# DhayaaAnbajagane/Baryonification

Hardware: AMD Instinct MI355X
Metric: halos/sec for BaryonifyShell NSIDE=1024 (1000000-halo synthetic catalog) (higher is better)
Workload: dtype f64 throughout in the parity-grade mode: f64 ring-row geometry, f64 pair math with 1e-11 elementary functions (fp32 seeds + one Newton step), f64 LDS accumulation, pix_offsets stored as two f32 arrays (hi + lo), f64 regrid geometry, f64 map

## Files before the change

### baryonification_amd/csrc/bfgx_kernels.hpp

```cpp
#pragma once
#include <hip/hip_runtime.h>
#include <stdint.h>
#include "bfgx_cosmo.hpp"
#include "bfgx_math.hpp"

namespace bfgx {

constexpr double kTwoPi    = 6.283185307179586476925286766559005768394;
constexpr double kHalfPi   = 1.570796326794896619231321691639751442099;
constexpr double kInvTwoPi = 1.0 / kTwoPi;
constexpr double kTwoThird = 2.0 / 3.0;
constexpr double kDeg2Rad  = kPi / 180.0;
constexpr double kRad2Deg  = 180.0 / kPi;

constexpr int kWave = 64;
constexpr int kWavesPerBlock = 4;
constexpr int kNC = 4;

enum { MODE_OFFSETS = 0, MODE_PAINT = 1, MODE_COUNT = 2 };

struct Hpx {
    int64_t nside, npix, ncap;
    double fact1, fact2;
};
// ... 3 lines not shown
    Hpx h;
    h.nside = nside;
    h.npix = 12 * nside * nside;
    h.ncap = 2 * nside * (nside - 1);
    h.fact2 = 4.0 / (double)h.npix;
    h.fact1 = (double)(nside << 1) * h.fact2;
    return h;
}

__device__ inline int64_t ring_above(const Hpx &h, double z)
{
    const double az = fabs(z);
    if (az <= kTwoThird) return (int64_t)((double)h.nside * (2.0 - 1.5 * z));
    const int64_t iring = (int64_t)((double)h.nside * sqrt(3.0 * (1.0 - az)));
    return (z > 0) ? iring : 4 * h.nside - iring - 1;
}

__device__ inline void ring_info_small(const Hpx &h, int64_t ring, int64_t &start, int64_t &nr, bool &shifted)
{
    if (ring < h.nside) {
        shifted = true; nr = 4 * ring; start = 2 * ring * (ring - 1);
    } else if (ring < 3 * h.nside) {
        shifted = ((ring - h.nside) & 1) == 0; nr = 4 * h.nside; start = h.ncap + (ring - h.nside) * nr;
    } else {
        const int64_t q = 4 * h.nside - ring;
        shifted = true; nr = 4 * q; start = h.npix - 2 * q * (q + 1);
    }
}

__device__ inline void ring_info2(const Hpx &h, int64_t ring, int64_t &start, int64_t &nr, double &theta, bool &shifted)
// ... 13 lines not shown

__device__ inline void ring_z_sth(const Hpx &h, int64_t ring, double &z, double &sth)
{
    if (ring < h.nside) {
        const double tmp = (double)(ring * ring) * h.fact2;
        z = 1.0 - tmp;
        sth = (z > 0.99) ? sqrt(tmp * (2.0 - tmp)) : sqrt((1.0 - z) * (1.0 + z));
    } else if (ring <= 3 * h.nside) {
        z = (double)(2 * h.nside - ring) * h.fact1;
        sth = sqrt((1.0 - z) * (1.0 + z));
    } else {
        const int64_t q = 4 * h.nside - ring;
        const double tmp = (double)(q * q) * h.fact2;
        z = tmp - 1.0;
        sth = (z < -0.99) ? sqrt(tmp * (2.0 - tmp)) : sqrt((1.0 - z) * (1.0 + z));
    }
}

__device__ inline int64_t isqrt64(int64_t v) { return (int64_t)sqrt((double)v + 0.5); }

__device__ inline void pix2loc(const Hpx &h, int64_t pix, double &z, double &sth, double &phi)
{
    if (pix < h.ncap) {
        const int64_t iring = (1 + isqrt64(1 + 2 * pix)) >> 1;
        const int64_t iphi = (pix + 1) - 2 * iring * (iring - 1);
        const double tmp = (double)(iring * iring) * h.fact2;
        z = 1.0 - tmp;
        sth = (z > 0.99) ? sqrt(tmp * (2.0 - tmp)) : sqrt((1.0 - z) * (1.0 + z));
        phi = ((double)iphi - 0.5) * kHalfPi / (double)iring;
    } else if (pix < h.npix - h.ncap) {
// ... 115 lines not shown
    if (!(dphi > 0.0)) return;
    const double sh = s.shifted ? 0.5 : 0.0;
    const double fnr = (double)s.nr * kInvTwoPi;
    const int64_t ip_lo = (int64_t)floor(fnr * (phi0 - dphi) - sh) + 1;
    const int64_t ip_hi = (int64_t)floor(fnr * (phi0 + dphi) - sh);
    int64_t c = ip_hi - ip_lo + 1;
    c = c < 0 ? 0 : (c > s.nr ? s.nr : c);
    s.cnt = (int)c;
    int64_t l = ip_lo;
    if (l < 0) l += s.nr;
    if (l >= s.nr) l -= s.nr;
    if (l < 0) l += s.nr;
    s.lo = (int)l;
}

__device__ inline void interp_neighbours(const Hpx &h, double theta, double phi, int32_t ring[4], int32_t k[4])
{
    int64_t pix[4]; double w[4];
    get_interpol<false>(h, theta, phi, pix, w);
    const double z = cos(theta);
    const int64_t ir1 = ring_above(h, z), ir2 = ir1 + 1;
    for (int q = 0; q < 4; ++q) {
        int64_t rg = (q < 2) ? ir1 : ir2;
        if (rg < 1) rg = 1;
        if (rg > 4 * h.nside - 1) rg = 4 * h.nside - 1;
        int64_t st, nr; bool sh;
        ring_info_small(h, rg, st, nr, sh);
        ring[q] = (int32_t)rg;
        k[q] = (int32_t)(pix[q] - st);
    }
}

struct DevTable {
    int32_t ndim;
    int32_t n[BFGX_MAX_DIM];
    const double *axis[BFGX_MAX_DIM];
// ... 69 lines not shown
    if (md.rho_type == 1) rho = b.rho_crit0 * b.Omega_m / (a * a * a);
    return cbrt(M / (4.18879020479 * md.Delta * rho));
}

__device__ inline int axis_find(const double *g, int n, double x)
{
    if (!(x >= g[0]) || !(x <= g[n - 1])) return -1;
    int lo = 0, hi = n - 1;
    while (hi - lo > 1) {
        const int mid = (lo + hi) >> 1;
        if (x >= g[mid]) lo = mid; else hi = mid;
    }
    return lo;
}

template <int NC>
__device__ inline bool table_corners(const DevTable &tab, const double *gz, const double *gm, double x0, double x1, const double *xe,
                                     double *wv, int32_t *ro)
{
    const int iz = axis_find(gz, tab.n[0], x0);
    const int im = axis_find(gm, tab.n[1], x1);
    constexpr int K = (NC == 4) ? 0 : (NC == 8 ? 1 : (NC == 16 ? 2 : (NC == 32 ? 3 : 4)));
    static_assert(NC == (4 << K), "NC = 4 * 2^K");
    int ip[K > 0 ? K : 1];
    double tp[K > 0 ? K : 1];
    bool oob = (iz < 0 || im < 0);
#pragma unroll
    for (int k = 0; k < K; ++k) {
        const double *g = tab.axis[3 + k];
        ip[k] = axis_find(g, tab.n[3 + k], xe[k]);
        tp[k] = 0.0;
        oob = oob || ip[k] < 0;
        if (ip[k] >= 0) tp[k] = (xe[k] - g[ip[k]]) / (g[ip[k] + 1] - g[ip[k]]);
    }
    if (!oob) {
        const double tz = (x0 - gz[iz]) / (gz[iz + 1] - gz[iz]);
        const double tm = (x1 - gm[im]) / (gm[im + 1] - gm[im]);
        const int nr = tab.n[2];
        for (int c = 0; c < NC; ++c) {
            const int bz = (c >> (K + 1)) & 1, bm = (c >> K) & 1;
            double w = (1.0 * (bz ? tz : 1.0 - tz)) * (bm ? tm : 1.0 - tm);
            int idx = (iz + bz) * tab.n[1] + im + bm;
#pragma unroll
            for (int k = 0; k < K; ++k) {
                const int b = (c >> (K - 1 - k)) & 1;
                w *= (b ? tp[k] : 1.0 - tp[k]);
                idx = idx * tab.n[3 + k] + ip[k] + b;
            }
            wv[c] = w;
            ro[c] = idx * nr;
        }
    } else {
        for (int c = 0; c < NC; ++c) { wv[c] = 0.0; ro[c] = 0; }
    }
    return oob;
}

struct Tiling {
    int32_t BR, W, nbands, ntiles;
    const int32_t *band_tile0;
    const int32_t *band_nphi;
    const int32_t *band_nrmin;
    const int32_t *tile_band;
    const int32_t *tile_order;
};

__device__ inline int tile_ks(int j, int nr, int nphi) { return (int)(((unsigned)j * (unsigned)nr + (unsigned)nphi - 1u) / (unsigned)nphi); }

__device__ inline int ring_len(const Hpx &h, int ring)
{
// ... 12 lines not shown
    int32_t _pad[2];
};

enum { kClsNone = 0, kClsNarrow = 1, kClsWide = 2 };

struct DiscSpan {
    int32_t fb, rfirst, rlast, allphi;
    int32_t fb_ring[4], fb_k[4];
    double flo, fhi;
};

template <typename F>
__device__ inline void for_each_tile(const Hpx &h, const Tiling &T, const DiscSpan &r, F &&f)
{
    if (r.fb) {
        int seen[4], ns = 0;
        for (int q = 0; q < 4; ++q) {
            const int b = (r.fb_ring[q] - 1) / T.BR;
            const int nphi = T.band_nphi[b];
            const int t = T.band_tile0[b] + (int)(((int64_t)r.fb_k[q] * nphi) / ring_len(h, r.fb_ring[q]));
            bool dup = false;
            for (int i = 0; i < ns; ++i) dup |= (seen[i] == t);
            if (!dup) { seen[ns++] = t; f(t); }
        }
        return;
    }
    if (r.rlast < r.rfirst) return;
    const int b0 = (r.rfirst - 1) / T.BR, b1 = (r.rlast - 1) / T.BR;
    for (int b = b0; b <= b1; ++b) {
        const int nphi = T.band_nphi[b], t0 = T.band_tile0[b];
        bool all = r.allphi || nphi == 1;
        int jlo = 0, jhi = nphi - 1;
        if (!all) {
            const double margin = 2.0 * (double)nphi / (double)T.band_nrmin[b] + 1e-6;
            jlo = (int)floor((double)nphi * r.flo - margin);
            jhi = (int)floor((double)nphi * r.fhi + margin);
            if (jhi - jlo + 1 >= nphi) { all = true; jlo = 0; jhi = nphi - 1; }
        }
        for (int jj = jlo; jj <= jhi; ++jj) {
            int j = jj % nphi;
            if (j < 0) j += nphi;
            f(t0 + j);
        }
    }
}

struct alignas(16) RowRec {
    double z0, s0, xa, cosr, phi0;
    int32_t rfirst, rlast;
    int32_t fb;
    int32_t _pad;
    double cut2;
};
struct FbRec { int32_t ring[4], k[4]; };

template <typename real>
struct alignas(16) PairRecT {
// ... 45 lines not shown
    RowRec *rowrec;
    void *pairrec;
    FbRec *fbrec;
    TileRef *tref;
    int32_t *cnt_a, *cnt_b, *cnt_w;
    int32_t *entries_a, *slow_list, *slow_cnt;
    float *work_est;
    int32_t cap_a;
    int32_t cnt_pad;
    int32_t fast;
    int32_t rec_all;
    int32_t ncell_m, nrm1;
    int64_t blk_rows, blk_stride;
};

template <int NC, typename real>
__device__ __forceinline__ void halo_prep_one(const DevModel &m, const Hpx &h, int64_t j, bool live, const double *gz, const double *gm,
                                              const double *__restrict__ M, const double *__restrict__ z,
                                              const double *__restrict__ ra, const double *__restrict__ dec,
                                              ExtraCols ex,
                                              const double *__restrict__ lnz1, const double *__restrict__ lnM,
                                              int fallback4, const Tiling &T, const PrepOut &o, int *s_nslow, float *s_work);

constexpr int kK0Occ = 4;
template <int NC, typename real>
__global__ void __launch_bounds__(256, kK0Occ)
halo_prep_kernel(DevModel m, Hpx h, int64_t nhalo,
                 const double *__restrict__ M, const double *__restrict__ z,
                 const double *__restrict__ ra, const double *__restrict__ dec,
                 ExtraCols ex,
                 const double *__restrict__ lnz1, const double *__restrict__ lnM,
                 int fallback4, Tiling T, PrepOut o)
{
    __shared__ int s_nslow;
    __shared__ float s_work;
    if (threadIdx.x == 0) { s_nslow = 0; s_work = 0.0f; }
    constexpr int kAxisLds = 128;
    __shared__ double ax_lds[2 * kAxisLds];
    const bool ax_in_lds = m.tab.n[0] <= kAxisLds && m.tab.n[1] <= kAxisLds;
    if (ax_in_lds) {
        for (int i = threadIdx.x; i < m.tab.n[0]; i += blockDim.x) ax_lds[i] = m.tab.axis[0][i];
        for (int i = threadIdx.x; i < m.tab.n[1]; i += blockDim.x) ax_lds[kAxisLds + i] = m.tab.axis[1][i];
        __syncthreads();
    }
    const double *gz = ax_in_lds ? ax_lds : m.tab.axis[0], *gm = ax_in_lds ? ax_lds + kAxisLds : m.tab.axis[1];
    constexpr int kBandLds = 1024;
    __shared__ int32_t band_lds[3 * kBandLds + 1];
    if (o.tref && T.nbands <= kBandLds) {
        for (int i = threadIdx.x; i <= T.nbands; i += blockDim.x) band_lds[i] = T.band_tile0[i];
        for (int i = threadIdx.x; i < T.nbands; i += blockDim.x) { band_lds[kBandLds + 1 + i] = T.band_nphi[i]; band_lds[2 * kBandLds + 1 + i] = T.band_nrmin[i]; }
        __syncthreads();
        T.band_tile0 = band_lds; T.band_nphi = band_lds + kBandLds + 1; T.band_nrmin = band_lds + 2 * kBandLds + 1;
    }
    __syncthreads();
    const int64_t j = (int64_t)blockIdx.x * blockDim.x + threadIdx.x;
    halo_prep_one<NC, real>(m, h, j < nhalo ? j : nhalo - 1, j < nhalo, gz, gm, M, z, ra, dec, ex, lnz1, lnM, fallback4, T, o, &s_nslow, &s_work);
    if (o.slow_cnt) {
        __syncthreads();
        if (threadIdx.x == 0) o.slow_cnt[blockIdx.x] = s_nslow;
        if (threadIdx.x == 0 && o.work_est) o.work_est[blockIdx.x] = s_work;
    }
}

template <int NC, typename real>
__device__ __forceinline__ void halo_prep_one(const DevModel &m, const Hpx &h, int64_t j, bool live, const double *gz, const double *gm,
                                              const double *__restrict__ M, const double *__restrict__ z,
                                              const double *__restrict__ ra, const double *__restrict__ dec,
                                              ExtraCols ex,
                                              const double *__restrict__ lnz1, const double *__restrict__ lnM,
                                              int fallback4, const Tiling &T, const PrepOut &o, int *s_nslow, float *s_work)
{
    HaloRec r;
    const int64_t jin = o.blk_rows > 0 ? (j / o.blk_rows) * o.blk_stride + (j % o.blk_rows) : j;
    const double M_j = M[jin], z_j = z[jin];
    const double a = 1.0 / (1.0 + z_j);
    const double R = dev_radius(m.bg_runner, m.md_runner, M_j, a);
    double D;
    {
        int i = (int)floor(z_j / m.da_step);
        i = max(0, min(i, kDaKnots - 2));
        const double t = z_j - (double)i * m.da_step;
        const double *c = m.da_coef + 4 * i;
        D = ((c[0] * t + c[1]) * t + c[2]) * t + c[3];
    }
    const double radius = R * m.eps_runner / D;

    const double theta = kHalfPi - dec[jin] * kDeg2Rad;
    const double phi = ra[jin] * kDeg2Rad;
    double st, ct, sp, cp;
    sincos_bounded(theta, st, ct);
    sincos_bounded(phi, sp, cp);
    const double thq = theta;
    double phq = phi - kTwoPi * floor(phi * kInvTwoPi);
    if (phq >= kTwoPi) phq -= kTwoPi;
    if (st == 0.0) phq = 0.0;
    r.z0 = ct;
    r.s0 = st;
    r.xa = 1.0 / sqrt((1.0 - r.z0) * (1.0 + r.z0));
    r.phi0 = phq;
    r.cph0 = cp; r.sph0 = sp;
    r.theta = theta; r.phi = phi;
    r.D = D; r.a = a;

    const int64_t nl4 = 4 * h.nside;
    bool pole = false;
    double sr_ = 0.0;
    const bool bad = !live || !(radius > 0.0) || !isfinite(radius) || !(theta >= 0.0) || !(theta <= kPi) || !isfinite(phi);
    if (bad) {
        r.cosr = 1.0; r.irmin = 1; r.irmax = 0; r.rfirst = 1; r.rlast = 0;
        r.z0 = 1.0; r.s0 = 0.0; r.xa = 1.0; r.phi0 = 0.0; r.cph0 = 1.0; r.sph0 = 0.0;
    } else if (radius >= kPi) {
        r.cosr = -1.0; r.irmin = (int32_t)nl4; r.irmax = 0; r.rfirst = 1; r.rlast = (int32_t)(nl4 - 1);
        pole = true;
    } else {
        double cr_;
        sincos_bounded(radius, sr_, cr_);
        r.cosr = cr_;
        const double rlat1 = thq - radius;
        const double rlat2 = thq + radius;
        int64_t irmin = ring_above(h, ct * cr_ + st * sr_) + 1;
        int64_t irmax = ring_above(h, ct * cr_ - st * sr_);
        if (irmax > nl4 - 1) irmax = nl4 - 1;
        r.irmin = (int32_t)irmin; r.irmax = (int32_t)irmax;
        r.rfirst = (int32_t)(((rlat1 <= 0) && (irmin > 1)) ? 1 : irmin);
        r.rlast = (int32_t)(((rlat2 >= kPi) && (irmax + 1 < nl4)) ? nl4 - 1 : irmax);
        pole = (rlat1 <= 0) || (rlat2 >= kPi);
    }
    double dmax;
    {
        const double sr = (radius >= kHalfPi) ? 1.0 : sr_;
        r.allphi = (pole || radius >= kHalfPi || !(sr < 0.999 * r.s0)) ? 1 : 0;
        const double xs = sr / r.s0, xs2 = xs * xs;
        const double as_small = xs * (1.0 + xs2 * (1.0 / 6.0 + xs2 * (3.0 / 40.0 + xs2 * (15.0 / 336.0 + xs2 * (105.0 / 3456.0)))));
        dmax = r.allphi ? kPi : (xs < 0.35 ? as_small * (1.0 + 2e-6) : asin(xs));
        r.flo = (phq - dmax) * kInvTwoPi;
        r.fhi = (phq + dmax) * kInvTwoPi;
    }

    r.fb = 0; r._pad = 0;
    for (int q = 0; q < 4; ++q) { r.fb_ring[q] = 0; r.fb_k[q] = 0; }
    if (fallback4 && !bad && (r.rlast - r.rfirst) < 8) {
        int total = 0;
        const int span = r.rlast - r.rfirst, mid = (r.rfirst + r.rlast) >> 1;
        for (int t = 0; t <= span && total < 4; ++t) {
            const int ring = mid + ((t & 1) ? ((t + 1) >> 1) : -(t >> 1));
            RowSpan s;
            disc_row(h, ring, r.z0, r.xa, r.cosr, r.phi0, r.irmin, r.irmax, s);
            total += s.cnt;
        }
        if (total < 4) {
            r.fb = 1;
            interp_neighbours(h, theta, phi, r.fb_ring, r.fb_k);
        }
    }

    int cls = kClsWide;
    bool geo_wide = false;
    if (bad) cls = kClsNone;
    else if (o.fast && NC == 4 && !r.allphi && dmax <= 0.40) {
        cls = kClsNarrow;
        if (r.fb) for (int q = 0; q < 4; ++q) if (r.fb_ring[q] < 16 || r.fb_ring[q] > (int)nl4 - 16) cls = kClsWide;
    }
    if (o.fast == 2 && NC == 4 && cls == kClsWide) { cls = kClsNarrow; geo_wide = true; }
    if (o.work_est) {
        float w = (cls == kClsNarrow) ? (r.fb ? 4.0f : (float)(radius * radius) * 0.25f * (float)h.npix) : 0.0f;
#pragma unroll
        for (int sft = kWave >> 1; sft > 0; sft >>= 1) w += __shfl_xor(w, sft, kWave);
        if ((threadIdx.x & (kWave - 1)) == 0) atomicAdd(s_work, w);
    }
    TileRef ref;
    RunSlot run[kRefMax];
    for (int i = 0; i < kRefMax; ++i) { run[i].base = 0; run[i].hr = 0; }
    ref.n = 0; ref.cls = cls; ref._pad[0] = ref._pad[1] = 0;
    for (int i = 0; i < kRefMax; ++i) { ref.few.tile[i] = 0; ref.few.slot[i] = 0; }
    if (o.tref) {
        DiscSpan ds;
        ds.fb = r.fb; ds.rfirst = r.rfirst; ds.rlast = r.rlast; ds.allphi = r.allphi; ds.flo = r.flo; ds.fhi = r.fhi;
        for (int q = 0; q < 4; ++q) { ds.fb_ring[q] = r.fb_ring[q]; ds.fb_k[q] = r.fb_k[q]; }
        int tl[kRefMax] = {0, 0, 0, 0};
        int nt = 0;
        if (cls != kClsNone) for_each_tile(h, T, ds, [&](int t) { if (nt < kRefMax) tl[nt] = t; ++nt; });
        ref.n = nt; ref.cls = cls; ref._pad[0] = ref._pad[1] = 0;
#pragma unroll
        for (int i = 0; i < kRefMax; ++i) {
            run[i] = wave_run_issue(o.cnt_a, o.entries_a ? tl[i] * o.cnt_pad : tl[i], nt <= kRefMax && i < nt && cls == kClsNarrow);
            if (nt <= kRefMax) { ref.few.tile[i] = (i < nt) ? tl[i] : 0; ref.few.slot[i] = 0; }
        }
        if (nt <= kRefMax) {
            for (int i = 0; i < kRefMax; ++i)
                if (i < nt && cls != kClsNarrow) atomicAdd(o.cnt_w + tl[i], 1);
        } else {
            ref.many.rfirst = r.rfirst; ref.many.rlast = r.rlast; ref.many.allphi = r.allphi; ref.many._p = 0;
            ref.many.flo = r.flo; ref.many.fhi = r.fhi;
            int32_t *cnt = (cls == kClsNarrow) ? o.cnt_b : o.cnt_w;
            for_each_tile(h, T, ds, [&](int t) { atomicAdd(cnt + t, 1); });
        }
    }
    const double Rmod = (m.same_model ? R : dev_radius(m.bg_model, m.md_model, M_j, a)) / a;
    r.rcut = m.tab.eps_model * Rmod;
    r.inv_a = 1.0 / a;
    const double x0 = lnz1 ? lnz1[jin] : fast_log(1.0 / a), x1 = lnM ? lnM[jin] : fast_log(M_j);
    r.lnoff = m.tab.rdelta ? (x0 - fast_log(Rmod)) : x0;
    double wv[NC];
    int32_t ro[NC];
    double xe[BFGX_MAX_EXTRA];
#pragma unroll
    for (int k = 0; k < BFGX_MAX_EXTRA; ++k) xe[k] = ((4 << k) < NC) ? ex.p[k][jin] : 0.0;
    const bool oob = table_corners<NC>(m.tab, gz, gm, x0, x1, xe, wv, ro);
    r.oob = oob ? 1 : 0;
    if (NC == 4) {
        for (int c = 0; c < 4; ++c) { r.w[c] = wv[c]; r.rowoff[c] = ro[c]; }
    } else {
        for (int c = 0; c < 4; ++c) { r.w[c] = 0.0; r.rowoff[c] = 0; }
        RowSetX rx;
        for (int c = 0; c < kNCmaxShell; ++c) { rx.w[c] = c < NC ? wv[c] : 0.0; rx.rowoff[c] = c < NC ? ro[c] : 0; }
        if (live) o.rowsx[j] = rx;
    }

    if (live && o.rec && (o.rec_all || cls == kClsWide)) o.rec[j] = r;
    if (cls == kClsNarrow) {
        RowRec rr;
        rr.z0 = r.z0; rr.s0 = r.s0; rr.xa = r.xa; rr.cosr = r.cosr; rr.phi0 = r.phi0;
        rr.rfirst = r.rfirst; rr.rlast = r.rlast; rr.fb = (r.fb ? 1 : 0) | (geo_wide ? 2 : 0); rr._pad = 0;
        const double cut = r.rcut * a / D;
        rr.cut2 = cut * cut;
        double sh, chh;
        sincos_bounded(0.5 * fmin(radius, kPi), sh, chh);
        const bool implied = (m.tab.logv != 0) || (!r.fb && cut >= 2.0 * sh * (1.0 + 1e-9));
        o.rowrec[j] = rr;
        PairRecT<real> pr;
        double scl = D * r.inv_a;
        if (m.tab.rdelta) scl /= Rmod;
        pr.scale2 = oob ? (real)1.0e30 : (real)(scl * scl);
        pr.cut2 = implied ? (real)0 : (real)(1.0 / rr.cut2);
        pr.aD = (real)(a / D);
        pr.cph0 = (real)r.cph0; pr.sph0 = (real)r.sph0;
        for (int c = 0; c < 4; ++c) pr.w[c] = (real)wv[c < NC ? c : 0];
        const int nr = o.nrm1 + 1, nm = o.ncell_m + 1;
        const int row0 = oob ? 0 : ro[0] / nr;
        const int iz = row0 / nm, im = row0 - iz * nm;
        pr.cell = (iz * o.ncell_m + im) * o.nrm1 * 8;
        pr.oob = oob ? 1 : 0;
        pr.hidx = (int32_t)j; pr._pad = 0;
        reinterpret_cast<PairRecT<real> *>(o.pairrec)[j] = pr;
        if (r.fb || geo_wide) {
            FbRec f;
            for (int q = 0; q < 4; ++q) { f.ring[q] = r.fb_ring[q]; f.k[q] = r.fb_k[q]; }
            if (!r.fb) { f.ring[0] = r.irmin; f.ring[1] = r.irmax; }
            o.fbrec[j] = f;
        }
    }
    if (o.tref) {
#pragma unroll
        for (int i = 0; i < kRefMax; ++i) {
            const int sl = wave_run_resolve(run[i]);
            if (ref.n <= kRefMax && ref.cls == kClsNarrow && i < ref.n) ref.few.slot[i] = sl;
        }
        bool slow = (ref.cls != kClsNone) && (ref.n > kRefMax || ref.cls != kClsNarrow);
        if (ref.cls == kClsNarrow && ref.n <= kRefMax) {
            for (int i = 0; i < kRefMax; ++i) if (i < ref.n) {
                const int sl = ref.few.slot[i];
                if (o.entries_a && sl < o.cap_a) o.entries_a[(int64_t)ref.few.tile[i] * o.cap_a + sl] = (int32_t)j;
                else if (o.entries_a) { ref.few.slot[i] = -1; atomicAdd(o.cnt_b + ref.few.tile[i], 1); slow = true; }
                else slow = true;
            }
        }
        if (live && (slow || !o.slow_list)) o.tref[j] = ref;
        if (slow && o.slow_list) o.slow_list[(int64_t)blockIdx.x * 256 + atomicAdd(s_nslow, 1)] = (int32_t)j;
    }
}

__global__ void __launch_bounds__(256)
disc_rings_kernel(DevModel m, Hpx h, int64_t nhalo, const double *__restrict__ M, const double *__restrict__ z,
                  const double *__restrict__ dec, int32_t *__restrict__ rings, int margin)
{
    const int64_t j = (int64_t)blockIdx.x * blockDim.x + threadIdx.x;
    if (j >= nhalo) return;
    const double M_j = M[j], z_j = z[j];
    const double a = 1.0 / (1.0 + z_j);
    const double R = dev_radius(m.bg_runner, m.md_runner, M_j, a);
    double D;
    {
        int i = (int)floor(z_j / m.da_step);
        i = max(0, min(i, kDaKnots - 2));
        const double t = z_j - (double)i * m.da_step;
        const double *c = m.da_coef + 4 * i;
        D = ((c[0] * t + c[1]) * t + c[2]) * t + c[3];
    }
    const double radius = R * m.eps_runner / D;
    const double theta = kHalfPi - dec[j] * kDeg2Rad;
    const int nl4 = (int)(4 * h.nside);
    int first = 1, last = 0;
    const bool bad = !(radius > 0.0) || !isfinite(radius) || !(theta >= 0.0) || !(theta <= kPi) || !(M_j > 0.0) || !isfinite(M_j) || !(z_j > -1.0);
    if (!bad) {
        if (radius >= kPi) { first = 1; last = nl4 - 1; }
        else {
            const double lo = fmax(theta - radius, 0.0), hi = fmin(theta + radius, kPi);
            first = (int)ring_above(h, cos(lo)) - 1;
            last = (int)ring_above(h, cos(hi)) + 2;
            first = max(1, first - 1); last = min(nl4 - 1, last + 1);
        }
        first = max(1, first - margin); last = min(nl4 - 1, last + margin);
    }
    rings[2 * j] = first; rings[2 * j + 1] = last;
// ... 85 lines not shown
    }
}
__global__ void __launch_bounds__(256)
route_step_kernel(RouteStepArgs s, DevModel m, Hpx h, int64_t n, int32_t *__restrict__ cursor)
{
    const RouteArgs &a = s.r;
    __shared__ int hist[kRouteMaxRanks], base[kRouteMaxRanks], taken[kRouteMaxRanks];
    const int tid = threadIdx.x;
    if (tid < kRouteMaxRanks) { hist[tid] = 0; taken[tid] = 0; }
    __syncthreads();
    const int64_t per = (n + gridDim.x - 1) / gridDim.x;
    const int64_t j0 = (int64_t)blockIdx.x * per, j1 = min(n, j0 + per);
    const int nl4 = (int)(4 * h.nside);
    auto ring_range = [&](int64_t j, int &first, int &last) {
        const double M_j = s.M[j], z_j = s.z[j];
        const double aa = 1.0 / (1.0 + z_j);
        const double R = dev_radius(m.bg_runner, m.md_runner, M_j, aa);
        double D;
        {
            int i = (int)floor(z_j / m.da_step);
            i = max(0, min(i, kDaKnots - 2));
            const double t = z_j - (double)i * m.da_step;
            const double *c = m.da_coef + 4 * i;
            D = ((c[0] * t + c[1]) * t + c[2]) * t + c[3];
        }
        const double radius = R * m.eps_runner / D;
        const double theta = kHalfPi - s.dec[j] * kDeg2Rad;
        first = 1; last = 0;
        const bool bad = !(radius > 0.0) || !isfinite(radius) || !(theta >= 0.0) || !(theta <= kPi) || !(M_j > 0.0) || !isfinite(M_j) || !(z_j > -1.0);
        if (bad) return;
        if (radius >= kPi) { first = 1; last = nl4 - 1; }
        else {
            const double lo = fmax(theta - radius, 0.0), hi = fmin(theta + radius, kPi);
            first = (int)ring_above(h, cos(lo)) - 1;
            last = (int)ring_above(h, cos(hi)) + 2;
            first = max(1, first - 1); last = min(nl4 - 1, last + 1);
        }
        first = max(1, first - s.margin); last = min(nl4 - 1, last + s.margin);
    };
    constexpr int kStash = 4096;
    __shared__ int2 stash[kStash];
// ... 899 lines not shown
```

### baryonification_amd/csrc/bfgx_scatter2.hpp

```cpp
#pragma once
#include "bfgx_kernels.hpp"
#include <type_traits>

namespace bfgx {

constexpr int kW2 = 8;
constexpr int kChunk2 = 16;
constexpr int kPlanePad = 11;

template <typename real> struct PMath;
__device__ inline float fma_(float a, float b, float c) { return __builtin_fmaf(a, b, c); }
__device__ inline double fma_(double a, double b, double c) { return __builtin_fma(a, b, c); }

template <> struct PMath<float> {
    static constexpr float kHuge = 1.0e37f;
    static __device__ inline float rsq(float x) { return __builtin_amdgcn_rsqf(x); }
    static __device__ inline float half_ln(float x) { return 0.34657359027997264f * __builtin_amdgcn_logf(x); }
    static __device__ inline float expv(float d) { return __builtin_amdgcn_exp2f(d * 1.4426950408889634f); }
    static __device__ inline void sin_omc(float x, float &sn, float &omc)
    {
        const float u = x * x;
        float ps = -1.0f / 5040.0f;
        ps = __builtin_fmaf(ps, u, 1.0f / 120.0f);
        ps = __builtin_fmaf(ps, u, -1.0f / 6.0f);
// ... 110 lines not shown
    PairRecT<real> pair[K1Cfg<real>::chunk];
    RowC2<real> rows[K1Cfg<real>::rowl];
    unsigned long long mask[K1Cfg<real>::rowl + 4];
    EntC2 ent[K1Cfg<real>::chunk];
    unsigned long long emask[K1Cfg<real>::chunk];
};

template <typename real>
__host__ __device__ inline size_t tile2_lds_bytes(int BR, int W, int ncomp)
{
    size_t a = (size_t)ncomp * ((size_t)BR * W + kPlanePad) * sizeof(double);
    a = (a + 15) & ~(size_t)15;
    return a + sizeof(Wave2Lds<real>) * kW2 + 16 + (sizeof(TileRow) + sizeof(RingC2<real>)) * (size_t)BR;
}

__constant__ double kAtanS1[6] = {1.62858201153657823623e-02, 4.97687799461593236017e-02, 6.66107313738753120669e-02,
                                  9.09088713343650656196e-02, 1.42857142725034663711e-01, 3.33333333333329318027e-01};
__constant__ double kAtanS2[5] = {-3.65315727442169155270e-02, -5.83357013379057348645e-02, -7.69187620504482999495e-02,
                                  -1.11111104054623557880e-01, -1.99999999998764832476e-01};
template <bool CMEM = false>
__device__ inline double atan_lt_7_16(double t)
{
    const double z = t * t, w = z * z;
    if (CMEM) {
        double s1 = kAtanS1[0], s2 = kAtanS2[0];
#pragma unroll
        for (int k = 1; k < 6; ++k) s1 = __builtin_fma(s1, w, kAtanS1[k]);
#pragma unroll
        for (int k = 1; k < 5; ++k) s2 = __builtin_fma(s2, w, kAtanS2[k]);
        return __builtin_fma(-t, __builtin_fma(z, s1, w * s2), t);
    }
    double s1 = 1.62858201153657823623e-02;
    s1 = __builtin_fma(s1, w, 4.97687799461593236017e-02);
    s1 = __builtin_fma(s1, w, 6.66107313738753120669e-02);
    s1 = __builtin_fma(s1, w, 9.09088713343650656196e-02);
    s1 = __builtin_fma(s1, w, 1.42857142725034663711e-01);
    s1 = __builtin_fma(s1, w, 3.33333333333329318027e-01);
    double s2 = -3.65315727442169155270e-02;
    s2 = __builtin_fma(s2, w, -5.83357013379057348645e-02);
    s2 = __builtin_fma(s2, w, -7.69187620504482999495e-02);
    s2 = __builtin_fma(s2, w, -1.11111104054623557880e-01);
    s2 = __builtin_fma(s2, w, -1.99999999998764832476e-01);
    return __builtin_fma(-t, __builtin_fma(z, s1, w * s2), t);
}

template <bool CMEM = false>
__device__ inline void disc_row_span_narrow(int nr, bool shifted, double z, double fnr, double z0, double xa, double cosr,
                                            double phi0, int &lo, int &cnt)
{
    lo = 0; cnt = 0;
    const double x = (cosr - z * z0) * xa;
    const double ysq = 1.0 - z * z - x * x;
    if (!(ysq > 0.0) || !(x > 0.0)) return;
    const double t = ysq * fast_rsq(ysq) * fast_rcp(x);
    const double dphi = atan_lt_7_16<CMEM>(t);
    if (!(dphi > 0.0)) return;
    const double sh = shifted ? 0.5 : 0.0;
    const int ip_lo = (int)floor(fnr * (phi0 - dphi) - sh) + 1;
    const int ip_hi = (int)floor(fnr * (phi0 + dphi) - sh);
    cnt = max(0, min(ip_hi - ip_lo + 1, nr));
    int l = ip_lo;
    if (l < 0) l += nr;
    if (l >= nr) l -= nr;
    if (l < 0) l += nr;
    lo = l;
}

__device__ __noinline__ bool exact_cut_test(const TileRow &tr, const RowRec &rr, int kloc)
{
    const int kk = tr.ks + kloc;
    const double xx = fold_dphi(__builtin_fma((double)kk + (tr.shifted ? 0.5 : 0.0), tr.dphi, -rr.phi0));
    double sh, ch;
    if (fabs(xx) <= 1.0) sincos_small(0.5 * xx, sh, ch);
    else sincos_bounded(0.5 * xx, sh, ch);
    const double s2 = 2.0 * sh * ch, o2 = 2.0 * sh * sh;
    const double wx = (tr.sth - rr.s0) - tr.sth * o2, wy = tr.sth * s2, wz = tr.z - rr.z0;
    return (wx * wx + wy * wy + wz * wz) < rr.cut2;
}

__device__ __noinline__ int2 disc_row_span_wide(const TileRow &tr, int ring, const RowRec &rr, const FbRec &fr)
{
// ... 846 lines not shown
```

Baseline: 911.7 million.

## Compact fallback-candidate halos into LDS work lists in the halo prep kernel

Restructures the halo prep kernel so the few-pixel fallback census and interp_neighbours run only on halos compacted into block-level LDS lists via wave ballots. The per-thread divergent fallback path becomes dense lane work. Several smaller edits come with it: 32-bit ring math, deferring the phi sincos, writing NC>4 table corners straight to global memory, cheaper tile dedup and wrap in for_each_tile, and a small-angle sincos. The cost is a large LDS struct and three extra block barriers per prep block.

```diff
diff --git a/baryonification_amd/csrc/bfgx_kernels.hpp b/baryonification_amd/csrc/bfgx_kernels.hpp
--- a/baryonification_amd/csrc/bfgx_kernels.hpp
+++ b/baryonification_amd/csrc/bfgx_kernels.hpp
@@ -41,6 +41,14 @@
     if (az <= kTwoThird) return (int64_t)((double)h.nside * (2.0 - 1.5 * z));
     const int64_t iring = (int64_t)((double)h.nside * sqrt(3.0 * (1.0 - az)));
     return (z > 0) ? iring : 4 * h.nside - iring - 1;
+}
+
+__device__ inline int ring_above32(const Hpx &h, double z)
+{
+    const double az = fabs(z);
+    if (az <= kTwoThird) return (int)((double)h.nside * (2.0 - 1.5 * z));
+    const int iring = (int)((double)h.nside * sqrt(3.0 * (1.0 - az)));
+    return (z > 0) ? iring : 4 * (int)h.nside - iring - 1;
 }
 
 __device__ inline void ring_info_small(const Hpx &h, int64_t ring, int64_t &start, int64_t &nr, bool &shifted)
@@ -84,6 +92,21 @@
         const double tmp = (double)(q * q) * h.fact2;
         z = tmp - 1.0;
         sth = (z < -0.99) ? sqrt(tmp * (2.0 - tmp)) : sqrt((1.0 - z) * (1.0 + z));
+    }
+}
+
+__device__ inline void ring_len_z(const Hpx &h, int ring, int &nr, bool &shifted, double &z)
+{
+    const int ns = (int)h.nside;
+    if (ring < ns) {
+        const double tmp = ((double)ring * (double)ring) * h.fact2;
+        z = 1.0 - tmp; nr = 4 * ring; shifted = true;
+    } else if (ring <= 3 * ns) {
+        z = (double)(2 * ns - ring) * h.fact1; nr = 4 * ns; shifted = ((ring - ns) & 1) == 0;
+    } else {
+        const int q = 4 * ns - ring;
+        const double tmp = ((double)q * (double)q) * h.fact2;
+        z = tmp - 1.0; nr = 4 * q; shifted = true;
     }
 }
 
@@ -229,12 +252,64 @@
     s.lo = (int)l;
 }
 
-__device__ inline void interp_neighbours(const Hpx &h, double theta, double phi, int32_t ring[4], int32_t k[4])
+__constant__ double kAtanS1[6] = {1.62858201153657823623e-02, 4.97687799461593236017e-02, 6.66107313738753120669e-02,
+                                  9.09088713343650656196e-02, 1.42857142725034663711e-01, 3.33333333333329318027e-01};
+__constant__ double kAtanS2[5] = {-3.65315727442169155270e-02, -5.83357013379057348645e-02, -7.69187620504482999495e-02,
+                                  -1.11111104054623557880e-01, -1.99999999998764832476e-01};
+template <bool CMEM = false>
+__device__ inline double atan_lt_7_16(double t)
+{
+    const double z = t * t, w = z * z;
+    if (CMEM) {
+        double s1 = kAtanS1[0], s2 = kAtanS2[0];
+#pragma unroll
+        for (int k = 1; k < 6; ++k) s1 = __builtin_fma(s1, w, kAtanS1[k]);
+#pragma unroll
+        for (int k = 1; k < 5; ++k) s2 = __builtin_fma(s2, w, kAtanS2[k]);
+        return __builtin_fma(-t, __builtin_fma(z, s1, w * s2), t);
+    }
+    double s1 = 1.62858201153657823623e-02;
+    s1 = __builtin_fma(s1, w, 4.97687799461593236017e-02);
+    s1 = __builtin_fma(s1, w, 6.66107313738753120669e-02);
+    s1 = __builtin_fma(s1, w, 9.09088713343650656196e-02);
+    s1 = __builtin_fma(s1, w, 1.42857142725034663711e-01);
+    s1 = __builtin_fma(s1, w, 3.33333333333329318027e-01);
+    double s2 = -3.65315727442169155270e-02;
+    s2 = __builtin_fma(s2, w, -5.83357013379057348645e-02);
+    s2 = __builtin_fma(s2, w, -7.69187620504482999495e-02);
+    s2 = __builtin_fma(s2, w, -1.11111104054623557880e-01);
+    s2 = __builtin_fma(s2, w, -1.99999999998764832476e-01);
+    return __builtin_fma(-t, __builtin_fma(z, s1, w * s2), t);
+}
+
+template <bool CMEM = false>
+__device__ inline void disc_row_span_narrow(int nr, bool shifted, double z, double fnr, double z0, double xa, double cosr,
+                                            double phi0, int &lo, int &cnt)
+{
+    lo = 0; cnt = 0;
+    const double x = (cosr - z * z0) * xa;
+    const double ysq = 1.0 - z * z - x * x;
+    if (!(ysq > 0.0) || !(x > 0.0)) return;
+    const double t = ysq * fast_rsq(ysq) * fast_rcp(x);
+    const double dphi = atan_lt_7_16<CMEM>(t);
+    if (!(dphi > 0.0)) return;
+    const double sh = shifted ? 0.5 : 0.0;
+    const int ip_lo = (int)floor(fnr * (phi0 - dphi) - sh) + 1;
+    const int ip_hi = (int)floor(fnr * (phi0 + dphi) - sh);
+    cnt = max(0, min(ip_hi - ip_lo + 1, nr));
+    int l = ip_lo;
+    if (l < 0) l += nr;
+    if (l >= nr) l -= nr;
+    if (l < 0) l += nr;
+    lo = l;
+}
+
+__device__ inline void interp_neighbours(const Hpx &h, double z, double theta, double phi, int32_t ring[4], int32_t k[4])
 {
     int64_t pix[4]; double w[4];
-    get_interpol<false>(h, theta, phi, pix, w);
-    const double z = cos(theta);
     const int64_t ir1 = ring_above(h, z), ir2 = ir1 + 1;
+    get_interpol_ring<false>(h, ir1, theta, phi, pix, w);
+#pragma unroll
     for (int q = 0; q < 4; ++q) {
         int64_t rg = (q < 2) ? ir1 : ir2;
         if (rg < 1) rg = 1;
@@ -334,9 +409,8 @@
     return lo;
 }
 
-template <int NC>
-__device__ inline bool table_corners(const DevTable &tab, const double *gz, const double *gm, double x0, double x1, const double *xe,
-                                     double *wv, int32_t *ro)
+template <int NC, typename F>
+__device__ inline bool table_corners_emit(const DevTable &tab, const double *gz, const double *gm, double x0, double x1, const double *xe, F &&emit)
 {
     const int iz = axis_find(gz, tab.n[0], x0);
     const int im = axis_find(gm, tab.n[1], x1);
@@ -367,13 +441,18 @@
                 w *= (b ? tp[k] : 1.0 - tp[k]);
                 idx = idx * tab.n[3 + k] + ip[k] + b;
             }
-            wv[c] = w;
-            ro[c] = idx * nr;
+            emit(c, w, idx * nr);
         }
     } else {
-        for (int c = 0; c < NC; ++c) { wv[c] = 0.0; ro[c] = 0; }
+        for (int c = 0; c < NC; ++c) emit(c, 0.0, 0);
     }
     return oob;
+}
+template <int NC>
+__device__ inline bool table_corners(const DevTable &tab, const double *gz, const double *gm, double x0, double x1, const double *xe,
+                                     double *wv, int32_t *ro)
+{
+    return table_corners_emit<NC>(tab, gz, gm, x0, x1, xe, [&](int c, double w, int32_t off) { wv[c] = w; ro[c] = off; });
 }
 
 struct Tiling {
@@ -416,14 +495,13 @@
 __device__ inline void for_each_tile(const Hpx &h, const Tiling &T, const DiscSpan &r, F &&f)
 {
     if (r.fb) {
-        int seen[4], ns = 0;
+        int s0 = -1, s1 = -1, s2 = -1;
+#pragma unroll
         for (int q = 0; q < 4; ++q) {
             const int b = (r.fb_ring[q] - 1) / T.BR;
             const int nphi = T.band_nphi[b];
-            const int t = T.band_tile0[b] + (int)(((int64_t)r.fb_k[q] * nphi) / ring_len(h, r.fb_ring[q]));
-            bool dup = false;
-            for (int i = 0; i < ns; ++i) dup |= (seen[i] == t);
-            if (!dup) { seen[ns++] = t; f(t); }
+            const int t = T.band_tile0[b] + (int)(((unsigned)r.fb_k[q] * (unsigned)nphi) / (unsigned)ring_len(h, r.fb_ring[q]));
+            if (t != s0 && t != s1 && t != s2) { s2 = s1; s1 = s0; s0 = t; f(t); }
         }
         return;
     }
@@ -434,15 +512,16 @@
         bool all = r.allphi || nphi == 1;
         int jlo = 0, jhi = nphi - 1;
         if (!all) {
-            const double margin = 2.0 * (double)nphi / (double)T.band_nrmin[b] + 1e-6;
+            const double margin = 2.0 * (double)nphi * fast_rcp((double)T.band_nrmin[b]) + 1e-6;
             jlo = (int)floor((double)nphi * r.flo - margin);
             jhi = (int)floor((double)nphi * r.fhi + margin);
             if (jhi - jlo + 1 >= nphi) { all = true; jlo = 0; jhi = nphi - 1; }
         }
+        int j = jlo % nphi;
+        if (j < 0) j += nphi;
         for (int jj = jlo; jj <= jhi; ++jj) {
-            int j = jj % nphi;
-            if (j < 0) j += nphi;
             f(t0 + j);
+            if (++j == nphi) j = 0;
         }
     }
 }
@@ -518,13 +597,68 @@
     int64_t blk_rows, blk_stride;
 };
 
+__device__ inline double halo_disc_radius(const DevModel &m, double M_j, double z_j, double &a, double &R, double &D)
+{
+    a = 1.0 / (1.0 + z_j);
+    R = dev_radius(m.bg_runner, m.md_runner, M_j, a);
+    int i = (int)floor(z_j / m.da_step);
+    i = max(0, min(i, kDaKnots - 2));
+    const double t = z_j - (double)i * m.da_step;
+    const double *c = m.da_coef + 4 * i;
+    D = ((c[0] * t + c[1]) * t + c[2]) * t + c[3];
+    return R * m.eps_runner / D;
+}
+
+struct K0Lds {
+    double z0[256], xa[256], cosr[256], phi0[256];
+    double theta[256], phi[256];
+    int32_t irmin[256], irmax[256], rfirst[256], rlast[256];
+    int32_t fb_k[4][256];
+    uint8_t flag[256];
+    uint8_t list1[256], list2[256];
+    int32_t n1, n2;
+};
+
+__device__ inline void wave_list_push(uint8_t *list, int32_t *count, bool push, int v)
+{
+    const unsigned long long bm = __ballot(push);
+    if (bm == 0ull) return;
+    const int below = (int)__builtin_amdgcn_mbcnt_hi((unsigned)(bm >> 32), __builtin_amdgcn_mbcnt_lo((unsigned)bm, 0u));
+    const int lane = (int)__builtin_amdgcn_mbcnt_hi(~0u, __builtin_amdgcn_mbcnt_lo(~0u, 0u));
+    int base = 0;
+    if (lane == 0) base = atomicAdd(count, (int)__popcll(bm));
+    base = __shfl(base, 0, kWave);
+    if (push) list[base + below] = (uint8_t)v;
+}
+
+__device__ inline int disc_census4(const Hpx &h, double z0, double xa, double cosr, double phi0, int irmin, int irmax, int rfirst, int rlast,
+                                   bool narrow)
+{
+    int total = 0;
+    const int span = rlast - rfirst, mid = (rfirst + rlast) >> 1;
+    for (int t = 0; t <= span && total < 4; ++t) {
+        const int ring = mid + ((t & 1) ? ((t + 1) >> 1) : -(t >> 1));
+        if (narrow) {
+            int nr, lo, cnt; bool shifted; double z;
+            ring_len_z(h, ring, nr, shifted, z);
+            disc_row_span_narrow(nr, shifted, z, (double)nr * kInvTwoPi, z0, xa, cosr, phi0, lo, cnt);
+            total += cnt;
+        } else {
+            RowSpan s;
+            disc_row(h, ring, z0, xa, cosr, phi0, irmin, irmax, s);
+            total += s.cnt;
+        }
+    }
+    return total;
+}
+
 template <int NC, typename real>
 __device__ __forceinline__ void halo_prep_one(const DevModel &m, const Hpx &h, int64_t j, bool live, const double *gz, const double *gm,
                                               const double *__restrict__ M, const double *__restrict__ z,
                                               const double *__restrict__ ra, const double *__restrict__ dec,
                                               ExtraCols ex,
                                               const double *__restrict__ lnz1, const double *__restrict__ lnM,
-                                              int fallback4, const Tiling &T, const PrepOut &o, int *s_nslow, float *s_work);
+                                              int fallback4, const Tiling &T, const PrepOut &o, int *s_nslow, float *s_work, K0Lds &L);
 
 constexpr int kK0Occ = 4;
 template <int NC, typename real>
@@ -538,7 +672,8 @@
 {
     __shared__ int s_nslow;
     __shared__ float s_work;
-    if (threadIdx.x == 0) { s_nslow = 0; s_work = 0.0f; }
+    __shared__ K0Lds s_ph;
+    if (threadIdx.x == 0) { s_nslow = 0; s_work = 0.0f; s_ph.n1 = 0; s_ph.n2 = 0; }
     constexpr int kAxisLds = 128;
     __shared__ double ax_lds[2 * kAxisLds];
     const bool ax_in_lds = m.tab.n[0] <= kAxisLds && m.tab.n[1] <= kAxisLds;
@@ -558,7 +693,7 @@
     }
     __syncthreads();
     const int64_t j = (int64_t)blockIdx.x * blockDim.x + threadIdx.x;
-    halo_prep_one<NC, real>(m, h, j < nhalo ? j : nhalo - 1, j < nhalo, gz, gm, M, z, ra, dec, ex, lnz1, lnM, fallback4, T, o, &s_nslow, &s_work);
+    halo_prep_one<NC, real>(m, h, j < nhalo ? j : nhalo - 1, j < nhalo, gz, gm, M, z, ra, dec, ex, lnz1, lnM, fallback4, T, o, &s_nslow, &s_work, s_ph);
     if (o.slow_cnt) {
         __syncthreads();
         if (threadIdx.x == 0) o.slow_cnt[blockIdx.x] = s_nslow;
@@ -572,28 +707,19 @@
                                               const double *__restrict__ ra, const double *__restrict__ dec,
                                               ExtraCols ex,
                                               const double *__restrict__ lnz1, const double *__restrict__ lnM,
-                                              int fallback4, const Tiling &T, const PrepOut &o, int *s_nslow, float *s_work)
+                                              int fallback4, const Tiling &T, const PrepOut &o, int *s_nslow, float *s_work, K0Lds &L)
 {
     HaloRec r;
+    const int tid = (int)threadIdx.x;
     const int64_t jin = o.blk_rows > 0 ? (j / o.blk_rows) * o.blk_stride + (j % o.blk_rows) : j;
     const double M_j = M[jin], z_j = z[jin];
-    const double a = 1.0 / (1.0 + z_j);
-    const double R = dev_radius(m.bg_runner, m.md_runner, M_j, a);
-    double D;
-    {
-        int i = (int)floor(z_j / m.da_step);
-        i = max(0, min(i, kDaKnots - 2));
-        const double t = z_j - (double)i * m.da_step;
-        const double *c = m.da_coef + 4 * i;
-        D = ((c[0] * t + c[1]) * t + c[2]) * t + c[3];
-    }
-    const double radius = R * m.eps_runner / D;
+    double a, R, D;
+    const double radius = halo_disc_radius(m, M_j, z_j, a, R, D);
 
     const double theta = kHalfPi - dec[jin] * kDeg2Rad;
     const double phi = ra[jin] * kDeg2Rad;
-    double st, ct, sp, cp;
+    double st, ct;
     sincos_bounded(theta, st, ct);
-    sincos_bounded(phi, sp, cp);
     const double thq = theta;
     double phq = phi - kTwoPi * floor(phi * kInvTwoPi);
     if (phq >= kTwoPi) phq -= kTwoPi;
@@ -602,19 +728,16 @@
     r.s0 = st;
     r.xa = 1.0 / sqrt((1.0 - r.z0) * (1.0 + r.z0));
     r.phi0 = phq;
-    r.cph0 = cp; r.sph0 = sp;
-    r.theta = theta; r.phi = phi;
-    r.D = D; r.a = a;
-
-    const int64_t nl4 = 4 * h.nside;
+
+    const int nl4 = 4 * (int)h.nside;
     bool pole = false;
     double sr_ = 0.0;
     const bool bad = !live || !(radius > 0.0) || !isfinite(radius) || !(theta >= 0.0) || !(theta <= kPi) || !isfinite(phi);
     if (bad) {
         r.cosr = 1.0; r.irmin = 1; r.irmax = 0; r.rfirst = 1; r.rlast = 0;
-        r.z0 = 1.0; r.s0 = 0.0; r.xa = 1.0; r.phi0 = 0.0; r.cph0 = 1.0; r.sph0 = 0.0;
+        r.z0 = 1.0; r.s0 = 0.0; r.xa = 1.0; r.phi0 = 0.0;
     } else if (radius >= kPi) {
-        r.cosr = -1.0; r.irmin = (int32_t)nl4; r.irmax = 0; r.rfirst = 1; r.rlast = (int32_t)(nl4 - 1);
+        r.cosr = -1.0; r.irmin = nl4; r.irmax = 0; r.rfirst = 1; r.rlast = nl4 - 1;
         pole = true;
     } else {
         double cr_;
@@ -622,40 +745,65 @@
         r.cosr = cr_;
         const double rlat1 = thq - radius;
         const double rlat2 = thq + radius;
-        int64_t irmin = ring_above(h, ct * cr_ + st * sr_) + 1;
-        int64_t irmax = ring_above(h, ct * cr_ - st * sr_);
+        const int irmin = ring_above32(h, ct * cr_ + st * sr_) + 1;
+        int irmax = ring_above32(h, ct * cr_ - st * sr_);
         if (irmax > nl4 - 1) irmax = nl4 - 1;
-        r.irmin = (int32_t)irmin; r.irmax = (int32_t)irmax;
-        r.rfirst = (int32_t)(((rlat1 <= 0) && (irmin > 1)) ? 1 : irmin);
-        r.rlast = (int32_t)(((rlat2 >= kPi) && (irmax + 1 < nl4)) ? nl4 - 1 : irmax);
+        r.irmin = irmin; r.irmax = irmax;
+        r.rfirst = ((rlat1 <= 0) && (irmin > 1)) ? 1 : irmin;
+        r.rlast = ((rlat2 >= kPi) && (irmax + 1 < nl4)) ? nl4 - 1 : irmax;
         pole = (rlat1 <= 0) || (rlat2 >= kPi);
     }
     double dmax;
     {
         const double sr = (radius >= kHalfPi) ? 1.0 : sr_;
         r.allphi = (pole || radius >= kHalfPi || !(sr < 0.999 * r.s0)) ? 1 : 0;
-        const double xs = sr / r.s0, xs2 = xs * xs;
+        const double xs = r.allphi ? 1.0 : sr * fast_rcp(r.s0), xs2 = xs * xs;
         const double as_small = xs * (1.0 + xs2 * (1.0 / 6.0 + xs2 * (3.0 / 40.0 + xs2 * (15.0 / 336.0 + xs2 * (105.0 / 3456.0)))));
         dmax = r.allphi ? kPi : (xs < 0.35 ? as_small * (1.0 + 2e-6) : asin(xs));
-        r.flo = (phq - dmax) * kInvTwoPi;
-        r.fhi = (phq + dmax) * kInvTwoPi;
-    }
-
-    r.fb = 0; r._pad = 0;
+    }
+
+    const bool cand = fallback4 && !bad && (r.rlast - r.rfirst) < 8;
+    L.flag[tid] = (!r.allphi && dmax <= 0.40) ? 2 : 0;
+    L.z0[tid] = r.z0; L.xa[tid] = r.xa; L.cosr[tid] = r.cosr; L.phi0[tid] = r.phi0; L.theta[tid] = theta; L.phi[tid] = phi;
+    if (cand) { L.irmin[tid] = r.irmin; L.irmax[tid] = r.irmax; L.rfirst[tid] = r.rfirst; L.rlast[tid] = r.rlast; }
+    wave_list_push(L.list1, &L.n1, cand, tid);
+    __syncthreads();
+
+    const int wave0 = __builtin_amdgcn_readfirstlane(tid & ~(kWave - 1));
+    if (wave0 < L.n1) {
+        bool few = false;
+        int slot = 0;
+        if (tid < L.n1) {
+            slot = L.list1[tid];
+            few = disc_census4(h, L.z0[slot], L.xa[slot], L.cosr[slot], L.phi0[slot], L.irmin[slot], L.irmax[slot], L.rfirst[slot], L.rlast[slot],
+                               (L.flag[slot] & 2) != 0) < 4;
+        }
+        wave_list_push(L.list2, &L.n2, few, slot);
+    }
+    __syncthreads();
+
+    if (tid < L.n2) {
+        const int slot = L.list2[tid];
+        int32_t fr[4], fk[4];
+        interp_neighbours(h, L.z0[slot], L.theta[slot], L.phi[slot], fr, fk);
+        L.irmin[slot] = fr[0]; L.irmax[slot] = fr[1]; L.rfirst[slot] = fr[2]; L.rlast[slot] = fr[3];
+#pragma unroll
+        for (int q = 0; q < 4; ++q) L.fb_k[q][slot] = fk[q];
+        L.flag[slot] |= 1;
+    }
+    __syncthreads();
+
+    r.z0 = L.z0[tid]; r.xa = L.xa[tid]; r.cosr = L.cosr[tid]; r.phi0 = L.phi0[tid]; r.theta = L.theta[tid]; r.phi = L.phi[tid];
+    r.D = D; r.a = a;
+    r.flo = (r.phi0 - dmax) * kInvTwoPi;
+    r.fhi = (r.phi0 + dmax) * kInvTwoPi;
+    r.fb = L.flag[tid] & 1; r._pad = 0;
+#pragma unroll
     for (int q = 0; q < 4; ++q) { r.fb_ring[q] = 0; r.fb_k[q] = 0; }
-    if (fallback4 && !bad && (r.rlast - r.rfirst) < 8) {
-        int total = 0;
-        const int span = r.rlast - r.rfirst, mid = (r.rfirst + r.rlast) >> 1;
-        for (int t = 0; t <= span && total < 4; ++t) {
-            const int ring = mid + ((t & 1) ? ((t + 1) >> 1) : -(t >> 1));
-            RowSpan s;
-            disc_row(h, ring, r.z0, r.xa, r.cosr, r.phi0, r.irmin, r.irmax, s);
-            total += s.cnt;
-        }
-        if (total < 4) {
-            r.fb = 1;
-            interp_neighbours(h, theta, phi, r.fb_ring, r.fb_k);
-        }
+    if (r.fb) {
+        r.fb_ring[0] = L.irmin[tid]; r.fb_ring[1] = L.irmax[tid]; r.fb_ring[2] = L.rfirst[tid]; r.fb_ring[3] = L.rlast[tid];
+#pragma unroll
+        for (int q = 0; q < 4; ++q) r.fb_k[q] = L.fb_k[q][tid];
     }
 
     int cls = kClsWide;
@@ -663,7 +811,7 @@
     if (bad) cls = kClsNone;
     else if (o.fast && NC == 4 && !r.allphi && dmax <= 0.40) {
         cls = kClsNarrow;
-        if (r.fb) for (int q = 0; q < 4; ++q) if (r.fb_ring[q] < 16 || r.fb_ring[q] > (int)nl4 - 16) cls = kClsWide;
+        if (r.fb) for (int q = 0; q < 4; ++q) if (r.fb_ring[q] < 16 || r.fb_ring[q] > nl4 - 16) cls = kClsWide;
     }
     if (o.fast == 2 && NC == 4 && cls == kClsWide) { cls = kClsNarrow; geo_wide = true; }
     if (o.work_est) {
@@ -674,16 +822,22 @@
     }
     TileRef ref;
     RunSlot run[kRefMax];
+#pragma unroll
     for (int i = 0; i < kRefMax; ++i) { run[i].base = 0; run[i].hr = 0; }
     ref.n = 0; ref.cls = cls; ref._pad[0] = ref._pad[1] = 0;
+#pragma unroll
     for (int i = 0; i < kRefMax; ++i) { ref.few.tile[i] = 0; ref.few.slot[i] = 0; }
     if (o.tref) {
         DiscSpan ds;
         ds.fb = r.fb; ds.rfirst = r.rfirst; ds.rlast = r.rlast; ds.allphi = r.allphi; ds.flo = r.flo; ds.fhi = r.fhi;
         for (int q = 0; q < 4; ++q) { ds.fb_ring[q] = r.fb_ring[q]; ds.fb_k[q] = r.fb_k[q]; }
-        int tl[kRefMax] = {0, 0, 0, 0};
-        int nt = 0;
-        if (cls != kClsNone) for_each_tile(h, T, ds, [&](int t) { if (nt < kRefMax) tl[nt] = t; ++nt; });
+        int tl0 = 0, tl1 = 0, tl2 = 0, tl3 = 0, nt = 0;
+        static_assert(kRefMax == 4, "the tile selects below are written out for 4");
+        if (cls != kClsNone) for_each_tile(h, T, ds, [&](int t) {
+            tl0 = (nt == 0) ? t : tl0; tl1 = (nt == 1) ? t : tl1; tl2 = (nt == 2) ? t : tl2; tl3 = (nt == 3) ? t : tl3;
+            ++nt;
+        });
+        const int tl[kRefMax] = {tl0, tl1, tl2, tl3};
         ref.n = nt; ref.cls = cls; ref._pad[0] = ref._pad[1] = 0;
 #pragma unroll
         for (int i = 0; i < kRefMax; ++i) {
@@ -691,6 +845,7 @@
             if (nt <= kRefMax) { ref.few.tile[i] = (i < nt) ? tl[i] : 0; ref.few.slot[i] = 0; }
         }
         if (nt <= kRefMax) {
+#pragma unroll
             for (int i = 0; i < kRefMax; ++i)
                 if (i < nt && cls != kClsNarrow) atomicAdd(o.cnt_w + tl[i], 1);
         } else {
@@ -700,26 +855,28 @@
             for_each_tile(h, T, ds, [&](int t) { atomicAdd(cnt + t, 1); });
         }
     }
+    if (bad) { r.cph0 = 1.0; r.sph0 = 0.0; }
+    else sincos_bounded(r.phi, r.sph0, r.cph0);
     const double Rmod = (m.same_model ? R : dev_radius(m.bg_model, m.md_model, M_j, a)) / a;
     r.rcut = m.tab.eps_model * Rmod;
     r.inv_a = 1.0 / a;
     const double x0 = lnz1 ? lnz1[jin] : fast_log(1.0 / a), x1 = lnM ? lnM[jin] : fast_log(M_j);
     r.lnoff = m.tab.rdelta ? (x0 - fast_log(Rmod)) : x0;
-    double wv[NC];
-    int32_t ro[NC];
+    double wv[4] = {0.0, 0.0, 0.0, 0.0};
+    int32_t ro[4] = {0, 0, 0, 0};
     double xe[BFGX_MAX_EXTRA];
 #pragma unroll
     for (int k = 0; k < BFGX_MAX_EXTRA; ++k) xe[k] = ((4 << k) < NC) ? ex.p[k][jin] : 0.0;
-    const bool oob = table_corners<NC>(m.tab, gz, gm, x0, x1, xe, wv, ro);
+    bool oob;
+    if (NC == 4) oob = table_corners<4>(m.tab, gz, gm, x0, x1, xe, wv, ro);
+    else {
+        RowSetX *rx = o.rowsx + j;
+        oob = table_corners_emit<NC>(m.tab, gz, gm, x0, x1, xe, [&](int c, double w, int32_t off) { if (live) { rx->w[c] = w; rx->rowoff[c] = off; } });
+        for (int c = NC; c < kNCmaxShell; ++c) if (live) { rx->w[c] = 0.0; rx->rowoff[c] = 0; }
+    }
     r.oob = oob ? 1 : 0;
-    if (NC == 4) {
-        for (int c = 0; c < 4; ++c) { r.w[c] = wv[c]; r.rowoff[c] = ro[c]; }
-    } else {
-        for (int c = 0; c < 4; ++c) { r.w[c] = 0.0; r.rowoff[c] = 0; }
-        RowSetX rx;
-        for (int c = 0; c < kNCmaxShell; ++c) { rx.w[c] = c < NC ? wv[c] : 0.0; rx.rowoff[c] = c < NC ? ro[c] : 0; }
-        if (live) o.rowsx[j] = rx;
-    }
+#pragma unroll
+    for (int c = 0; c < 4; ++c) { r.w[c] = wv[c]; r.rowoff[c] = ro[c]; }
 
     if (live && o.rec && (o.rec_all || cls == kClsWide)) o.rec[j] = r;
     if (cls == kClsNarrow) {
@@ -729,7 +886,8 @@
         const double cut = r.rcut * a / D;
         rr.cut2 = cut * cut;
         double sh, chh;
-        sincos_bounded(0.5 * fmin(radius, kPi), sh, chh);
+        if (radius <= 1.0) sincos_small(0.5 * radius, sh, chh);
+        else sincos_bounded(0.5 * fmin(radius, kPi), sh, chh);
         const bool implied = (m.tab.logv != 0) || (!r.fb && cut >= 2.0 * sh * (1.0 + 1e-9));
         o.rowrec[j] = rr;
         PairRecT<real> pr;
@@ -739,7 +897,7 @@
         pr.cut2 = implied ? (real)0 : (real)(1.0 / rr.cut2);
         pr.aD = (real)(a / D);
         pr.cph0 = (real)r.cph0; pr.sph0 = (real)r.sph0;
-        for (int c = 0; c < 4; ++c) pr.w[c] = (real)wv[c < NC ? c : 0];
+        for (int c = 0; c < 4; ++c) pr.w[c] = (real)wv[c];
         const int nr = o.nrm1 + 1, nm = o.ncell_m + 1;
         const int row0 = oob ? 0 : ro[0] / nr;
         const int iz = row0 / nm, im = row0 - iz * nm;
@@ -762,6 +920,7 @@
         }
         bool slow = (ref.cls != kClsNone) && (ref.n > kRefMax || ref.cls != kClsNarrow);
         if (ref.cls == kClsNarrow && ref.n <= kRefMax) {
+#pragma unroll
             for (int i = 0; i < kRefMax; ++i) if (i < ref.n) {
                 const int sl = ref.few.slot[i];
                 if (o.entries_a && sl < o.cap_a) o.entries_a[(int64_t)ref.few.tile[i] * o.cap_a + sl] = (int32_t)j;
@@ -781,17 +940,8 @@
     const int64_t j = (int64_t)blockIdx.x * blockDim.x + threadIdx.x;
     if (j >= nhalo) return;
     const double M_j = M[j], z_j = z[j];
-    const double a = 1.0 / (1.0 + z_j);
-    const double R = dev_radius(m.bg_runner, m.md_runner, M_j, a);
-    double D;
-    {
-        int i = (int)floor(z_j / m.da_step);
-        i = max(0, min(i, kDaKnots - 2));
-        const double t = z_j - (double)i * m.da_step;
-        const double *c = m.da_coef + 4 * i;
-        D = ((c[0] * t + c[1]) * t + c[2]) * t + c[3];
-    }
-    const double radius = R * m.eps_runner / D;
+    double a, R, D;
+    const double radius = halo_disc_radius(m, M_j, z_j, a, R, D);
     const double theta = kHalfPi - dec[j] * kDeg2Rad;
     const int nl4 = (int)(4 * h.nside);
     int first = 1, last = 0;
@@ -907,17 +1057,8 @@
     const int nl4 = (int)(4 * h.nside);
     auto ring_range = [&](int64_t j, int &first, int &last) {
         const double M_j = s.M[j], z_j = s.z[j];
-        const double aa = 1.0 / (1.0 + z_j);
-        const double R = dev_radius(m.bg_runner, m.md_runner, M_j, aa);
-        double D;
-        {
-            int i = (int)floor(z_j / m.da_step);
-            i = max(0, min(i, kDaKnots - 2));
-            const double t = z_j - (double)i * m.da_step;
-            const double *c = m.da_coef + 4 * i;
-            D = ((c[0] * t + c[1]) * t + c[2]) * t + c[3];
-        }
-        const double radius = R * m.eps_runner / D;
+        double aa, R, D;
+        const double radius = halo_disc_radius(m, M_j, z_j, aa, R, D);
         const double theta = kHalfPi - s.dec[j] * kDeg2Rad;
         first = 1; last = 0;
         const bool bad = !(radius > 0.0) || !isfinite(radius) || !(theta >= 0.0) || !(theta <= kPi) || !(M_j > 0.0) || !isfinite(M_j) || !(z_j > -1.0);
diff --git a/baryonification_amd/csrc/bfgx_scatter2.hpp b/baryonification_amd/csrc/bfgx_scatter2.hpp
--- a/baryonification_amd/csrc/bfgx_scatter2.hpp
+++ b/baryonification_amd/csrc/bfgx_scatter2.hpp
@@ -148,57 +148,6 @@
     return a + sizeof(Wave2Lds<real>) * kW2 + 16 + (sizeof(TileRow) + sizeof(RingC2<real>)) * (size_t)BR;
 }
 
-__constant__ double kAtanS1[6] = {1.62858201153657823623e-02, 4.97687799461593236017e-02, 6.66107313738753120669e-02,
-                                  9.09088713343650656196e-02, 1.42857142725034663711e-01, 3.33333333333329318027e-01};
-__constant__ double kAtanS2[5] = {-3.65315727442169155270e-02, -5.83357013379057348645e-02, -7.69187620504482999495e-02,
-                                  -1.11111104054623557880e-01, -1.99999999998764832476e-01};
-template <bool CMEM = false>
-__device__ inline double atan_lt_7_16(double t)
-{
-    const double z = t * t, w = z * z;
-    if (CMEM) {
-        double s1 = kAtanS1[0], s2 = kAtanS2[0];
-#pragma unroll
-        for (int k = 1; k < 6; ++k) s1 = __builtin_fma(s1, w, kAtanS1[k]);
-#pragma unroll
-        for (int k = 1; k < 5; ++k) s2 = __builtin_fma(s2, w, kAtanS2[k]);
-        return __builtin_fma(-t, __builtin_fma(z, s1, w * s2), t);
-    }
-    double s1 = 1.62858201153657823623e-02;
-    s1 = __builtin_fma(s1, w, 4.97687799461593236017e-02);
-    s1 = __builtin_fma(s1, w, 6.66107313738753120669e-02);
-    s1 = __builtin_fma(s1, w, 9.09088713343650656196e-02);
-    s1 = __builtin_fma(s1, w, 1.42857142725034663711e-01);
-    s1 = __builtin_fma(s1, w, 3.33333333333329318027e-01);
-    double s2 = -3.65315727442169155270e-02;
-    s2 = __builtin_fma(s2, w, -5.83357013379057348645e-02);
-    s2 = __builtin_fma(s2, w, -7.69187620504482999495e-02);
-    s2 = __builtin_fma(s2, w, -1.11111104054623557880e-01);
-    s2 = __builtin_fma(s2, w, -1.99999999998764832476e-01);
-    return __builtin_fma(-t, __builtin_fma(z, s1, w * s2), t);
-}
-
-template <bool CMEM = false>
-__device__ inline void disc_row_span_narrow(int nr, bool shifted, double z, double fnr, double z0, double xa, double cosr,
-                                            double phi0, int &lo, int &cnt)
-{
-    lo = 0; cnt = 0;
-    const double x = (cosr - z * z0) * xa;
-    const double ysq = 1.0 - z * z - x * x;
-    if (!(ysq > 0.0) || !(x > 0.0)) return;
-    const double t = ysq * fast_rsq(ysq) * fast_rcp(x);
-    const double dphi = atan_lt_7_16<CMEM>(t);
-    if (!(dphi > 0.0)) return;
-    const double sh = shifted ? 0.5 : 0.0;
-    const int ip_lo = (int)floor(fnr * (phi0 - dphi) - sh) + 1;
-    const int ip_hi = (int)floor(fnr * (phi0 + dphi) - sh);
-    cnt = max(0, min(ip_hi - ip_lo + 1, nr));
-    int l = ip_lo;
-    if (l < 0) l += nr;
-    if (l >= nr) l -= nr;
-    if (l < 0) l += nr;
-    lo = l;
-}
 
 __device__ __noinline__ bool exact_cut_test(const TileRow &tr, const RowRec &rr, int kloc)
 {
```

Result: no change. 913.4 million, median of 2 (+0.2%).
